# YuePanEdward/MULLS

Hardware: NVIDIA H100
Metric: scan-pair registrations/sec (120k-pt 64-beam) (higher is better)
Workload: dtype f32 geometry / f64 accumulation

## Files before the change

mulls_b200/csrc/kernels_ingest.cuh:

```cuda
#pragma once
#include "device_math.cuh"
#include "device_types.cuh"

namespace mulls {

template <bool kUndistort, bool kNormals>
__device__ __forceinline__ void load_input_point(const PairConst &pc, uint32_t seg, uint32_t local, float4 &pos, float4 &nrm) {
    const bool is_src = seg >= kNumClasses;
    const int cls = seg % kNumClasses;
    const bool undistort = kUndistort && is_src && pc.undistort && cls != MULLS_VERTEX;
    float x, y, z, intensity = 0.0f, curvature = 0.0f;
    float nx = 0.0f, ny = 0.0f, nz = 0.0f;
    const uint32_t fmt = pc.in_fmt[seg];
    if (fmt == 0u) {
        const float4 *in = pc.in_ptr[seg] + 3 * (size_t)local;
        const float4 a = in[0];
        x = a.x, y = a.y, z = a.z;
        if (kNormals) {
            const float4 b = in[1];
            const float4 c = in[2];
            nx = b.x, ny = b.y, nz = b.z;
            intensity = c.x, curvature = c.y;
        } else if (undistort) {
            curvature = reinterpret_cast<const float *>(in + 2)[1];
// ... 304 lines not shown
        uint32_t v = 0;
        if (i < total) v = A.ps[i / kNumSegs].seg_count[i % kNumSegs];
        uint32_t incl = v;
        for (int o = 1; o < 32; o <<= 1) {
            uint32_t t = __shfl_up_sync(0xffffffffu, incl, o);
            if ((threadIdx.x & 31) >= o) incl += t;
        }
        if ((threadIdx.x & 31) == 31) warp_sums[threadIdx.x >> 5] = incl;
        __syncthreads();
        if (threadIdx.x < 32) {
            uint32_t w = (threadIdx.x < (blockDim.x >> 5)) ? warp_sums[threadIdx.x] : 0;
            uint32_t wi = w;
            for (int o = 1; o < 32; o <<= 1) {
                uint32_t t = __shfl_up_sync(0xffffffffu, wi, o);
                if (threadIdx.x >= o) wi += t;
            }
            warp_sums[threadIdx.x] = wi - w;
        }
        __syncthreads();
        const uint32_t excl = carry + warp_sums[threadIdx.x >> 5] + incl - v;
        if (i < total) A.ps[i / kNumSegs].seg_start[i % kNumSegs] = excl;
        __syncthreads();
        if (threadIdx.x == blockDim.x - 1) carry = excl + v;
        __syncthreads();
    }
    for (int p = threadIdx.x; p < n_pairs; p += blockDim.x) {
        PairState &ps = A.ps[p];
        const PairConst &pc = A.pc[p];
        for (int c = 0; c < kNumClasses; ++c) {
            ps.n_tgt[c] = (int)ps.seg_count[c];
            ps.n_src[c] = (int)ps.seg_count[kNumClasses + c];
            ps.n_src_g[c] = ps.n_src[c];
            ps.n_corr[c] = 0;
            ps.n_corr_last[c] = 0;
        }
        int cnt = 0;
        if (pc.used[MULLS_PILLAR]) cnt += ps.n_src[MULLS_PILLAR];
        if (pc.used[MULLS_FACADE]) cnt += ps.n_src[MULLS_FACADE];
        if (pc.used[MULLS_BEAM]) cnt += ps.n_src[MULLS_BEAM];
        ps.source_feature_points_count = cnt;
    }
}

__device__ __forceinline__ int cell_top(const uint64_t *keys, uint32_t i, uint64_t kcur) {
    if (kcur == ~0ull || ((uint32_t)(kcur >> 36) % kNumSegs) >= kNumClasses) return -1;
    if (i == 0) return kMaxLevels - 1;
    const uint64_t kprev = keys[i - 1];
    if ((kprev >> 36) != (kcur >> 36)) return kMaxLevels - 1;
    const uint64_t diff = (kcur ^ kprev) & ((1ull << 36) - 1);
    if (diff == 0) return -1;
    return (63 - __clzll((long long)diff)) / 3;
}

template <bool kUndistort>
__global__ void __launch_bounds__(256) k_gather(DeviceArrays A, const uint64_t *keys, const uint32_t *vals, uint32_t n_total) {
    const uint32_t i = blockIdx.x * blockDim.x + threadIdx.x;
    const uint64_t key = i < n_total ? keys[i] : ~0ull;
    const uint32_t sg = (uint32_t)(key >> 36);
    const uint32_t pair = sg / kNumSegs, seg = sg % kNumSegs;
    const int top = cell_top(keys, i, key);
    const int cnt = top < 0 ? 0 : min(top, A.ps[pair].n_levels - 1) + 1;
    const bool is_tgt = key != ~0ull && seg < kNumClasses;
    const unsigned grp = __match_any_sync(0xffffffffu, is_tgt ? sg : 0xffffffffu);
    if (grp == 0xffffffffu) {
        const int tot = __reduce_add_sync(0xffffffffu, cnt);
        if ((threadIdx.x & 31) == 0 && tot > 0) atomicAdd(&A.ps[pair].hash_entries[seg], (unsigned)tot);
    } else if (cnt > 0) {
        atomicAdd(&A.ps[pair].hash_entries[seg], (unsigned)cnt);
    }
    if (key == ~0ull) return;
    const PairConst &pc = A.pc[pair];
    float4 pos, nrm;
    load_input_point<kUndistort, true>(pc, seg, vals[i] - pc.in_off[seg], pos, nrm);
    const uint32_t local = i - A.ps[pair].seg_start[seg];
    if (seg < kNumClasses) {
        const uint32_t d = pc.tgt_base[seg] + local;
        A.tgt_pos[d] = pos;
        A.tgt_nrm[d] = nrm;
    } else {
        const uint32_t d = pc.src_base[seg - kNumClasses] + local;
        if (pc.sharded) nrm.w = __int_as_float(__float_as_int(nrm.w) + (int)pc.src_index_base[seg - kNumClasses]);
        A.src_pos[0][d] = pos;
        A.src_nrm[0][d] = nrm;
        A.src_prevj[0][d] = -1;
        A.src_cert[0][d] = make_float4(0.f, 0.f, 0.f, 0.f);
    }
}

__device__ __forceinline__ void hash_insert(HashEntry *table, uint32_t hmask, uint32_t klo, uint32_t khi, uint32_t children,
                                            uint32_t start, uint32_t count) {
    uint32_t slot = cell_hash(klo, khi) & hmask;
    const unsigned long long packed = (unsigned long long)klo | ((unsigned long long)(khi | (children << 16)) << 32);
    while (true) {
        unsigned long long *kp = reinterpret_cast<unsigned long long *>(&table[slot]);
        if (atomicCAS(kp, 0ull, packed) == 0ull) {
            *reinterpret_cast<uint2 *>(&table[slot].start) = make_uint2(start, count);
            return;
        }
        slot = (slot + 1) & hmask;
    }
}

__device__ __forceinline__ uint32_t cell_end(const uint64_t *keys, uint32_t b, uint32_t hi, uint64_t p, int shift) {
    uint32_t in = b, out = hi, step = 1;
    while (in + step < hi) {
        if ((keys[in + step] >> shift) != p) {
            out = in + step;
            break;
        }
        in += step;
        step <<= 1;
    }
    while (out - in > 1) {
        const uint32_t mid = in + (out - in) / 2;
        if ((keys[mid] >> shift) == p) in = mid;
        else out = mid;
    }
    return out;
}

__global__ void __launch_bounds__(256) k_hash_build(DeviceArrays A, const uint64_t *keys, uint32_t n_total) {
    const uint32_t i = blockIdx.x * blockDim.x + threadIdx.x;
    if (i >= n_total || A.hash_used[1]) return;
    const uint64_t kcur = keys[i];
    const int top = cell_top(keys, i, kcur);
    if (top < 0) return;
    const uint32_t sg = (uint32_t)(kcur >> 36);
    const uint32_t pair = sg / kNumSegs, cls = sg % kNumSegs;
    const PairState &ps = A.ps[pair];
    const int L = ps.n_levels;
    const uint32_t seg_begin = ps.seg_start[cls], seg_end = seg_begin + ps.seg_count[cls];
    HashEntry *table = A.hash + ps.hash_base[cls];
    const uint32_t hmask = ps.hash_mask[cls];
    const uint64_t m = kcur & ((1ull << 36) - 1);
    const uint32_t x0 = compact12(m), y0 = compact12(m >> 1), z0 = compact12(m >> 2);
    uint32_t end = cell_end(keys, i, seg_end, kcur, 0);
    for (int l = 0; l <= top && l < L; ++l) {
        uint32_t children = 0;
        if (l > 0) {
            const int shift = 3 * l;
            const uint64_t p = kcur >> shift;
            children = 1u << ((kcur >> (shift - 3)) & 7u);
            while (end < seg_end) {
                const uint64_t k = keys[end];
                if ((k >> shift) != p) break;
                children |= 1u << ((k >> (shift - 3)) & 7u);
                end = cell_end(keys, end, seg_end, k >> (shift - 3), shift - 3);
            }
        }
        const uint32_t x = x0 >> l, y = y0 >> l, z = z0 >> l;
        hash_insert(table, hmask, cell_key_lo(x, y, z), cell_key_hi(z, l), children, i - seg_begin, end - i);
    }
}

constexpr uint64_t kHashSlack = 4;
__device__ __forceinline__ uint64_t hash_table_cap(int attempt, uint32_t cells) {
    const uint64_t want = (attempt == 0) ? kHashSlack * cells : (attempt == 1) ? 2ull * cells : (5ull * cells) / 4 + 1;
    uint64_t cap = 16;
    while (cap < want) cap <<= 1;
    return cap;
}
__global__ void k_hash_layout(DeviceArrays A, int n_pairs) {
    if (threadIdx.x != 0 || blockIdx.x != 0) return;
    for (int attempt = 0; attempt < 3; ++attempt) {
        uint64_t used = 0;
        bool overflow = false;
        for (int p = 0; p < n_pairs && !overflow; ++p) {
            PairState &ps = A.ps[p];
// ... 41 lines not shown
```

mulls_b200/csrc/kernels_iterate.cuh:

```cuda
#pragma once
#include <cooperative_groups.h>

#include "device_math.cuh"
#include "device_types.cuh"
#include "kernels_ingest.cuh"

namespace mulls {

__device__ __forceinline__ bool chunk_in_run(const DeviceArrays &A) { return blockIdx.x < (unsigned)A.ctl->n_it_chunks; }
__device__ __forceinline__ int loop_buf(const DeviceArrays &A, int buf) { return buf >= 0 ? buf : (A.ctl->it & 1); }
__device__ __forceinline__ mulls_icp_trace *trace_of(const DeviceArrays &A, uint32_t pair) {
    return (A.trace && A.ctl->trace_on) ? &A.trace[pair] : nullptr;
}

template <class Body>
__device__ __forceinline__ void for_each_live_chunk(const DeviceArrays &A, int parity, int which, Body body) {
    __shared__ uint32_t s_fetch;
    LoopCtl &ctl = *A.ctl;
    const uint32_t n = ctl.n_live[parity];
    const uint32_t *list = A.live_chunks + (size_t)parity * A.live_stride;
    for (;;) {
        __syncthreads();
        if (threadIdx.x == 0) s_fetch = atomicAdd(&ctl.work[which], 1u);
        __syncthreads();
        const uint32_t w = s_fetch;
        if (w >= n) break;
        body(list[w]);
    }
}

__device__ __forceinline__ void append_live_chunks(const DeviceArrays &A, int parity, uint32_t first, uint32_t count, uint32_t base) {
    uint32_t *list = A.live_chunks + (size_t)parity * A.live_stride;
    for (uint32_t k = threadIdx.x; k < count; k += blockDim.x) list[base + k] = first + k;
}

__global__ void __launch_bounds__(256) k_live_init(DeviceArrays A) {
    LoopCtl &ctl = *A.ctl;
    const uint32_t chunk = blockIdx.x * blockDim.x + threadIdx.x;
    bool live = false;
    if (chunk < (uint32_t)ctl.n_it_chunks) {
        const ChunkDesc cd = A.it_chunks[chunk];
        live = (int)cd.first < A.ps[cd.pair].n_src[cd.seg];
    }
    const unsigned m = __ballot_sync(0xffffffffu, live);
    if (!m) return;
    const int lane = threadIdx.x & 31;
    uint32_t base = 0;
    if (lane == 0) base = atomicAdd(&ctl.n_live[0], (unsigned)__popc(m));
    base = __shfl_sync(0xffffffffu, base, 0);
    if (live) A.live_chunks[base + __popc(m & ((1u << lane) - 1u))] = chunk;
}

constexpr int kStartLevel0 = 5;
constexpr int kLeafCount = 32;
constexpr int kDeferFromIter = 3;
constexpr float kReseedCells = 4.0f;

__device__ __forceinline__ GridView grid_of(const DeviceArrays &A, const PairConst &pc, const PairState &ps, int c) {
    GridView g;
    g.table = A.hash + ps.hash_base[c];
    g.mask = ps.hash_mask[c];
    g.pos = A.tgt_pos + pc.tgt_base[c];
    g.nrm = A.tgt_nrm + pc.tgt_base[c];
    g.ox = ps.origin[0], g.oy = ps.origin[1], g.oz = ps.origin[2];
    g.h0 = ps.h0, g.inv_h0 = ps.inv_h0;
    g.n_levels = ps.n_levels;
    g.leaf_count = kLeafCount;
    g.level_slack2 = 1.002001f;
    return g;
}

constexpr int kShootK = 10;

__device__ __forceinline__ void load_and_advance(DeviceArrays &A, const PairState &ps, int buf, uint32_t gi, bool valid,
                                                 float4 &p, float4 &n) {
    p = A.src_pos[buf][gi];
    n = A.src_nrm[buf][gi];
    if (valid && ps.iter > 0) {
        const double *t = ps.T_inc;
        const double px = p.x, py = p.y, pz = p.z, qx = n.x, qy = n.y, qz = n.z;
        p.x = (float)(t[0] * px + t[1] * py + t[2] * pz + t[3]);
        p.y = (float)(t[4] * px + t[5] * py + t[6] * pz + t[7]);
        p.z = (float)(t[8] * px + t[9] * py + t[10] * pz + t[11]);
        n.x = (float)(t[0] * qx + t[1] * qy + t[2] * qz);
        n.y = (float)(t[4] * qx + t[5] * qy + t[6] * qz);
        n.z = (float)(t[8] * qx + t[9] * qy + t[10] * qz);
        A.src_pos[buf][gi] = p;
        A.src_nrm[buf][gi] = n;
    }
}

__device__ __forceinline__ bool shoots(const PairConst &pc, int c) {
    return pc.normal_shooting && (c == MULLS_GROUND || c == MULLS_FACADE || c == MULLS_ROOF);
}

constexpr int kKeepFromIter = 3;

struct SearchFrame {
    GridView g;
    double max_dist_sqr;
    float r2_prune;
    bool defer;
};
__device__ __forceinline__ SearchFrame search_frame(const DeviceArrays &A, const PairConst &pc, const PairState &ps, int c) {
    SearchFrame f;
    f.g = grid_of(A, pc, ps, c);
    const float max_distance_f = 2.5f * ps.thre;
    f.max_dist_sqr = (double)max_distance_f * (double)max_distance_f;
    f.r2_prune = (float)f.max_dist_sqr * 1.0001f;
    f.defer = ps.iter >= kDeferFromIter;
    return f;
}

__device__ __forceinline__ void search_finish(DeviceArrays &A, const PairConst &pc, int c, uint32_t gi, int best_j, float best_d2,
                                              double max_dist_sqr, float orig_index_bits) {
    if (best_j >= 0 && !((double)best_d2 <= max_dist_sqr)) best_j = -1;
    if (best_j >= 0) {
        atomicMin(&A.claim[pc.tgt_base[c] + best_j], (unsigned)__float_as_int(orig_index_bits));
    }
    A.nn_idx[gi] = best_j;
    A.nn_d2[gi] = best_d2;
}

template <class Bounds>
__device__ __forceinline__ void search_one(DeviceArrays &A, const PairConst &pc, int c, int buf, uint32_t gi, const float4 p,
                                           float orig_bits, const SearchFrame &f, bool write_cert) {
    NoStats st;
    int best_j = -1;
    float best_d2 = INFINITY;
    const int pj = A.src_prevj[buf][gi];
    if (pj >= 0) {
        const float4 q = __ldg(&f.g.pos[pj]);
        best_d2 = flann_l2(p.x, p.y, p.z, q.x, q.y, q.z);
        best_j = pj;
    }
    {
        const float rs = kReseedCells * f.g.h0;
        if (best_j < 0 || best_d2 > rs * rs) {
            float d2 = INFINITY;
            int j = -1;
            walk_greedy_seed(f.g, p.x, p.y, p.z, kStartLevel0, d2, j, st);
            if (j >= 0 && d2 < best_d2) best_d2 = d2, best_j = j;
        }
    }
    const float cert2 = nn_search_walk_b<Bounds>(f.g, p.x, p.y, p.z, f.r2_prune, kStartLevel0, f.defer, best_d2, best_j, st);
    if (write_cert) A.src_cert[buf][gi] = make_float4(p.x, p.y, p.z, sqrtf(cert2));
    search_finish(A, pc, c, gi, best_j, best_d2, f.max_dist_sqr, orig_bits);
}

template <class Bounds>
__device__ __forceinline__ void search_quarter(DeviceArrays &A, int buf, uint32_t chunk, uint32_t sub, bool write_cert) {
    const ChunkDesc cd = A.it_chunks[chunk];
    const PairConst &pc = A.pc[cd.pair];
    const PairState &ps = A.ps[cd.pair];
    if (ps.status != kRunning || A.hash_used[1]) return;
    const int c = (int)cd.seg;
    const int ns = ps.n_src[c], nt = ps.n_tgt[c], nsg = ps.n_src_g[c];
    if ((int)cd.first >= ns) return;
    if (shoots(pc, c)) return;
    const uint32_t local = cd.first + 32u * sub + (threadIdx.x & 31u);
    const bool valid = (int)local < ns;
    const uint32_t gi = pc.src_base[c] + (valid ? local : 0);
    float4 p, n;
    load_and_advance(A, ps, buf, gi, valid, p, n);
    if (!valid) return;
    if (!(pc.used[c] && nsg >= 3 && nt >= 3)) {
        A.nn_idx[gi] = -1;
        A.nn_d2[gi] = INFINITY;
        return;
    }
    const SearchFrame f = search_frame(A, pc, ps, c);
    search_one<Bounds>(A, pc, c, buf, gi, p, n.w, f, write_cert);
}

__device__ __forceinline__ void search_keep_chunk(DeviceArrays &A, int buf, uint32_t chunk, uint8_t *need_list, uint32_t *n_need) {
    const ChunkDesc cd = A.it_chunks[chunk];
    const PairConst &pc = A.pc[cd.pair];
    const PairState &ps = A.ps[cd.pair];
    if (ps.status != kRunning || A.hash_used[1]) return;
    const int c = (int)cd.seg;
    const int ns = ps.n_src[c], nt = ps.n_tgt[c], nsg = ps.n_src_g[c];
    if ((int)cd.first >= ns) return;
    if (shoots(pc, c)) return;
    const int lane = threadIdx.x & 31;
    const bool active = pc.used[c] && nsg >= 3 && nt >= 3;
    const SearchFrame f = search_frame(A, pc, ps, c);
    if (threadIdx.x == 0) *n_need = 0u;
    __syncthreads();
    {
        const uint32_t local = cd.first + threadIdx.x;
        const bool valid = (int)local < ns;
        const uint32_t gi = pc.src_base[c] + (valid ? local : 0);
        float4 p, n;
        load_and_advance(A, ps, buf, gi, valid, p, n);
        bool need = false;
        if (valid) {
            if (!active) {
                A.nn_idx[gi] = -1;
                A.nn_d2[gi] = INFINITY;
            } else {
                need = true;
                const int pj = A.src_prevj[buf][gi];
                const float4 ce = A.src_cert[buf][gi];
                if (pj >= 0 && ce.w > 0.0f) {
                    const float4 q = __ldg(&f.g.pos[pj]);
                    const float d1 = flann_l2(p.x, p.y, p.z, q.x, q.y, q.z);
                    const float mv = flann_l2(p.x, p.y, p.z, ce.x, ce.y, ce.z);
                    if ((sqrtf(d1) + sqrtf(mv)) * 1.0001f + 3e-5f < ce.w * 0.9999f) {
                        search_finish(A, pc, c, gi, pj, d1, f.max_dist_sqr, n.w);
                        need = false;
                    }
                }
            }
        }
        const unsigned m = __ballot_sync(0xffffffffu, need);
        uint32_t base = 0;
        if (lane == 0 && m) base = atomicAdd(n_need, (uint32_t)__popc(m));
        base = __shfl_sync(0xffffffffu, base, 0);
        if (need) need_list[base + __popc(m & ((1u << lane) - 1u))] = (uint8_t)threadIdx.x;
    }
    __syncthreads();
    if (threadIdx.x < *n_need) {
        const uint32_t gi = pc.src_base[c] + cd.first + need_list[threadIdx.x];
        const float4 p = A.src_pos[buf][gi];
        search_one<WalkBounds>(A, pc, c, buf, gi, p, A.src_nrm[buf][gi].w, f, true);
    }
}

constexpr int kSearchBlocksPerSm = 10;
__device__ __forceinline__ int search_mode_of(int it) { return it >= kKeepFromIter ? 2 : (it == kKeepFromIter - 1 ? 1 : 0); }

template <int kMode>
__global__ void __launch_bounds__(kIterBlock, kSearchBlocksPerSm) k_search(DeviceArrays A, int buf, int it) {
    buf = loop_buf(A, buf);
    if (it < 0) it = A.ctl->it;
    if (blockIdx.x == 0 && threadIdx.x == 0) {
        LoopCtl &ctl = *A.ctl;
        ctl.work[1] = ctl.work[2] = ctl.work[3] = 0u;
        ctl.n_live[buf ^ 1] = 0u;
    }
    if (search_mode_of(it) != kMode) return;
    if (kMode == 2) {
        __shared__ uint8_t s_need[kIterBlock];
        __shared__ uint32_t s_n_need;
        for_each_live_chunk(A, buf, 0, [&](uint32_t chunk) { search_keep_chunk(A, buf, chunk, s_need, &s_n_need); });
    } else {
        const uint32_t n_units = (kIterBlock / 32) * A.ctl->n_live[buf];
        const uint32_t *list = A.live_chunks + (size_t)buf * A.live_stride;
        for (;;) {
            uint32_t u = 0;
            if ((threadIdx.x & 31) == 0) u = atomicAdd(&A.ctl->work[0], 1u);
            u = __shfl_sync(0xffffffffu, u, 0);
            if (u >= n_units) break;
            if (kMode == 1) search_quarter<WalkBounds>(A, buf, list[u / (kIterBlock / 32)], u % (kIterBlock / 32), true);
            else search_quarter<NoBounds>(A, buf, list[u / (kIterBlock / 32)], u % (kIterBlock / 32), false);
            __syncwarp();
        }
    }
}

__device__ __forceinline__ void search_shoot_chunk(DeviceArrays &A, int buf, uint32_t chunk) {
    const ChunkDesc cd = A.it_chunks[chunk];
    const PairConst &pc = A.pc[cd.pair];
    const PairState &ps = A.ps[cd.pair];
    if (ps.status != kRunning || A.hash_used[1]) return;
    const int c = (int)cd.seg;
    const int ns = ps.n_src[c], nt = ps.n_tgt[c], nsg = ps.n_src_g[c];
    if ((int)cd.first >= ns || !shoots(pc, c)) return;
    const uint32_t local = cd.first + threadIdx.x;
    const bool valid = (int)local < ns;
    const uint32_t gi = pc.src_base[c] + (valid ? local : 0);
    float4 p, n;
    load_and_advance(A, ps, buf, gi, valid, p, n);
    if (!valid) return;
    if (!(pc.used[c] && nsg >= 3 && nt >= 3)) {
        A.nn_idx[gi] = -1;
        A.nn_d2[gi] = INFINITY;
        return;
    }
    const GridView g = grid_of(A, pc, ps, c);
    const float max_distance_f = 2.5f * ps.thre;
    int sj = -1;
    float sd2 = INFINITY;
    KnnList<kShootK> kl;
    knn_search(g, p.x, p.y, p.z, kStartLevel0, kShootK, kl);
    double min_dist = 1.7976931348623157e308;
    for (int t = 0; t < kl.n; ++t) {
        const float4 q = __ldg(&g.pos[kl.j[t]]);
        const float ptx = q.x - p.x, pty = q.y - p.y, ptz = q.z - p.z;
        const double Nx = n.x, Ny = n.y, Nz = n.z, Vx = ptx, Vy = pty, Vz = ptz;
        const double Cx = Ny * Vz - Nz * Vy, Cy = Nz * Vx - Nx * Vz, Cz = Nx * Vy - Ny * Vx;
        const double dist = Cx * Cx + (Cy * Cy + Cz * Cz);
        if (dist < min_dist) {
            min_dist = dist;
            sj = kl.j[t];
            sd2 = kl.d2[t];
        }
    }
    if (sj >= 0 && min_dist > (double)max_distance_f) sj = -1;
    if (sj >= 0) atomicMin(&A.claim[pc.tgt_base[c] + sj], (unsigned)__float_as_int(n.w));
    A.nn_idx[gi] = sj;
    A.nn_d2[gi] = sd2;
}
__global__ void __launch_bounds__(kIterBlock) k_search_shoot(DeviceArrays A, int buf) {
    buf = loop_buf(A, buf);
    for_each_live_chunk(A, buf, 3, [&](uint32_t chunk) { search_shoot_chunk(A, buf, chunk); });
}

__device__ __forceinline__ void resolve_body(DeviceArrays &A, int buf, uint32_t chunk) {
    const ChunkDesc cd = A.it_chunks[chunk];
    const PairConst &pc = A.pc[cd.pair];
    PairState &ps = A.ps[cd.pair];
    if (ps.status != kRunning) return;
    const int c = (int)cd.seg;
    const int ns = ps.n_src[c], nt = ps.n_tgt[c], nsg = ps.n_src_g[c];
    const uint32_t local = cd.first + threadIdx.x;
    const bool valid = (int)local < ns;
    const bool active = pc.used[c] && nsg >= 3 && nt >= 3;
    const bool dedup = active && nsg >= kDedupMinSrc;
    bool kept = false, pass = false;
    if (valid) {
        const uint32_t gi = pc.src_base[c] + local;
        const int j = A.nn_idx[gi];
        const bool matched = active && j >= 0;
        bool corr = matched;
        kept = true;
        if (dedup) {
            const float4 n = A.src_nrm[buf][gi];
            const bool winner = matched && A.claim[pc.tgt_base[c] + j] == (unsigned)__float_as_int(n.w);
            kept = winner;
            corr = winner;
        }
        if (corr) {
            const float d2 = A.nn_d2[gi];
            pass = d2 < ps.thre * ps.thre;
            if (pass && c != MULLS_VERTEX) {
                const float4 n = A.src_nrm[buf][gi];
                const float4 m = A.tgt_nrm[pc.tgt_base[c] + j];
                const double dot = (double)n.x * (double)m.x + (double)n.y * (double)m.y + (double)n.z * (double)m.z;
                const float cos_angle = (float)fabs(dot);
                if ((double)cos_angle < pc.cos_thre) pass = false;
            }
        }
        A.flags[gi] = (uint8_t)((kept ? 1 : 0) | (pass ? 2 : 0));
    }
    const unsigned kb = __ballot_sync(0xffffffffu, kept);
    const unsigned pb = __ballot_sync(0xffffffffu, pass);
    __shared__ unsigned s_kept[kIterBlock / 32], s_pass[kIterBlock / 32];
    if ((threadIdx.x & 31) == 0) {
        s_kept[threadIdx.x >> 5] = __popc(kb);
        s_pass[threadIdx.x >> 5] = __popc(pb);
    }
    __syncthreads();
    if (threadIdx.x == 0) {
        unsigned k = 0, p = 0;
        for (int w = 0; w < kIterBlock / 32; ++w) {
            k += s_kept[w];
            p += s_pass[w];
        }
        A.blk_kept[chunk] = k;
        if (p) atomicAdd(&ps.n_corr[c], p);
    }
}
__global__ void __launch_bounds__(kIterBlock) k_resolve(DeviceArrays A, int buf) {
    buf = loop_buf(A, buf);
    for_each_live_chunk(A, buf, 1, [&](uint32_t chunk) { resolve_body(A, buf, chunk); });
}

template <class Sink>
__device__ __forceinline__ void terms_pt2pl(const float4 p, const float pi, const float4 q, const float4 qn,
                                            float weight, int iter_num, bool dist_w, bool resid_w, bool inten_w,
                                            float window, Sink t, float &w_out) {
    const float px = p.x, py = p.y, pz = p.z, qx = q.x, qy = q.y, qz = q.z;
    const float ntx = qn.x, nty = qn.y, ntz = qn.z;
    float w = weight;
    const float a = ntz * py - nty * pz;
    const float b = ntx * pz - ntz * px;
    const float c = nty * px - ntx * py;
    const float d = ntx * qx + nty * qy + ntz * qz - ntx * px - nty * py - ntz * pz;
    const float dist = sqrtf(qx * qx + qy * qy + qz * qz);
    if (dist_w) w = w * weight_by_dist_adaptive(dist, iter_num);
    if (resid_w) w = w * weight_by_residual(fabsf(d), window);
    if (inten_w) w = w * weight_by_intensity((float)((double)pi + 0.0001), (float)((double)q.w + 0.0001));
    w_out = w;
    t[0] = w * ntx * ntx;
    t[1] = w * ntx * nty;
    t[2] = w * ntx * ntz;
    t[3] = w * a * ntx;
    t[4] = w * b * ntx;
    t[5] = w * c * ntx;
    t[6] = w * nty * nty;
    t[7] = w * nty * ntz;
    t[8] = w * a * nty;
    t[9] = w * b * nty;
    t[10] = w * c * nty;
    t[11] = w * ntz * ntz;
    t[12] = w * a * ntz;
    t[13] = w * b * ntz;
    t[14] = w * c * ntz;
    t[15] = w * a * a;
    t[16] = w * a * b;
    t[17] = w * a * c;
    t[18] = w * b * b;
    t[19] = w * b * c;
    t[20] = w * c * c;
    t[21] = w * d * ntx;
    t[22] = w * d * nty;
    t[23] = w * d * ntz;
    t[24] = w * d * a;
    t[25] = w * d * b;
    t[26] = w * d * c;
}

__device__ __forceinline__ int diag_index(int j) {
    const int d[6] = {0, 6, 11, 15, 18, 20};
    return d[j];
}

template <class Sink>
__device__ __forceinline__ void terms_pt2li(const float4 p, const float pi, const float4 q, const float4 qv,
                                            float weight, int iter_num, bool dist_w, bool resid_w, bool inten_w,
                                            float window, Sink t, float &w_out) {
    const float px = p.x, py = p.y, pz = p.z, qx = q.x, qy = q.y, qz = q.z;
    const float vx = qv.x, vy = qv.y, vz = qv.z;
    const float dx = px - qx, dy = py - qy, dz = pz - qz;
    double Am[3][6], bv[3];
    Am[0][0] = 0;
    Am[0][1] = (double)(-vz);
    Am[0][2] = (double)vy;
    Am[0][3] = (double)(vy * py + vz * pz);
    Am[0][4] = (double)(-vy * px);
    Am[0][5] = (double)(-vz * px);
    Am[1][0] = (double)vz;
    Am[1][1] = 0;
    Am[1][2] = (double)(-vx);
    Am[1][3] = (double)(-vx * py);
    Am[1][4] = (double)(vz * pz + vx * px);
    Am[1][5] = (double)(-vz * py);
    Am[2][0] = (double)(-vy);
    Am[2][1] = (double)vx;
    Am[2][2] = 0;
    Am[2][3] = (double)(-vx * pz);
    Am[2][4] = (double)(-vy * pz);
    Am[2][5] = (double)(vx * px + vy * py);
    bv[0] = (double)(-vy * dz + vz * dy);
    bv[1] = (double)(-vz * dx + vx * dz);
    bv[2] = (double)(-vx * dy + vy * dx);
// ... 180 lines not shown
        for (int r = 0; r < 3; ++r)
            for (int cc = 0; cc < 3; ++cc)
                cof[6 * (3 + r) + cc] = J[r][0] * inv[6 * 3 + cc] + J[r][1] * inv[6 * 4 + cc] + J[r][2] * inv[6 * 5 + cc];
    }
    double *Tt = ps.T_inc;
    construct_trans_a(x, Tt);
    const double ts_norm = sqrt(Tt[3] * Tt[3] + Tt[7] * Tt[7] + Tt[11] * Tt[11]);
    const double rs_angle = fabs(rotation_angle(Tt));
    if (ts_norm > (double)pc.max_t || rs_angle > (double)pc.max_r) {
        ps.code = -1;
        ps.status = kDone;
        pair_left_running(A);
        return;
    }
    mat4_mul(Tt, ps.T_total, Tmp);
    for (int k = 0; k < 16; ++k) ps.T_total[k] = Tmp[k];
    if (i == pc.max_iter - 1 || (i > 2 && ts_norm < (double)pc.conv_t && rs_angle < (double)pc.conv_r)) {
        ps.status = kNeedPosterior;
        ps.final_buf = buf_written;
        pair_left_running(A);
        return;
    }
    ps.iter = i + 1;
}

__device__ __forceinline__ void accumulate_body(DeviceArrays &A, int buf, uint32_t chunk) {
    const ChunkDesc cd = A.it_chunks[chunk];
    const PairConst &pc = A.pc[cd.pair];
    PairState &ps = A.ps[cd.pair];
    if (ps.status != kRunning) return;
    const int c = (int)cd.seg;
    const int ns = ps.n_src[c];
    const uint32_t local = cd.first + threadIdx.x;
    const bool valid = (int)local < ns;
    const int lane = threadIdx.x & 31, warp = threadIdx.x >> 5;
    constexpr int kWarps = kIterBlock / 32;
    __shared__ double s_terms[27 * kIterBlock];
    __shared__ uint32_t s_off[kWarps + 1];
    __shared__ uint32_t s_base;

    if ((int)cd.first >= ns) return;
    uint32_t dst_local = 0;
    uint8_t fl = 0;
    uint32_t gi = 0;
    bool kept = false, pass = false;
    struct Column {
        double *base;
        __device__ __forceinline__ double &operator[](int k) const { return base[k * kIterBlock]; }
    } t = {s_terms + threadIdx.x};
    {
        uint32_t acc = 0;
        const uint32_t first_chunk = pc.class_chunk_begin[c];
        for (uint32_t b = first_chunk + threadIdx.x; b < chunk; b += kIterBlock) acc += A.blk_kept[b];
        for (int o = 16; o > 0; o >>= 1) acc += __shfl_xor_sync(0xffffffffu, acc, o);
        if (lane == 0) s_off[warp] = acc;
        __syncthreads();
        if (threadIdx.x == 0) {
            uint32_t tt = 0;
            for (int w = 0; w < kWarps; ++w) tt += s_off[w];
            s_base = tt;
        }
        __syncthreads();
    }
    if (valid) {
        gi = pc.src_base[c] + local;
        fl = A.flags[gi];
    }
    kept = (fl & 1) != 0, pass = (fl & 2) != 0;
    const unsigned kb = __ballot_sync(0xffffffffu, kept);
    if (lane == 0) s_off[warp] = __popc(kb);
    __syncthreads();
    if (threadIdx.x == 0) {
        uint32_t run = 0;
        for (int w = 0; w < kWarps; ++w) {
            const uint32_t tt = s_off[w];
            s_off[w] = run;
            run += tt;
        }
        s_off[kWarps] = run;
    }
    __syncthreads();
    dst_local = s_base + s_off[warp] + __popc(kb & ((1u << lane) - 1u));

    float w_store = 0.0f;
    int j = -1;
    float4 p = make_float4(0, 0, 0, 0), n = make_float4(0, 0, 0, 0);
    float d2 = 0.0f;
    if (valid) {
        p = A.src_pos[buf][gi];
        n = A.src_nrm[buf][gi];
        j = A.nn_idx[gi];
        d2 = A.nn_d2[gi];
        if (j >= 0) A.claim[pc.tgt_base[c] + j] = kClaimFree;
    }
    uint32_t n_corr[kNumClasses];
#pragma unroll
    for (int k = 0; k < kNumClasses; ++k) n_corr[k] = ps.n_corr[k];
    float ratio_unused;
    const bool few = too_few(pc, ps, n_corr, ratio_unused);
    if (pass && !few) {
        const float4 q = A.tgt_pos[pc.tgt_base[c] + j];
        const float4 qn = A.tgt_nrm[pc.tgt_base[c] + j];
        const int it = ps.iter;
        const bool resid_w = pc.w_residual && it > 2;
        const bool dist_w = pc.w_dist != 0, inten_w = pc.w_intensity != 0;
        if (c == MULLS_GROUND || c == MULLS_FACADE || c == MULLS_ROOF) {
            const float wc = (c == MULLS_FACADE) ? 1.0f : balanced_ground_weight(pc, n_corr);
            terms_pt2pl(p, p.w, q, qn, wc, it, dist_w, resid_w, inten_w, pc.win_pt2pl, t, w_store);
        } else if (c == MULLS_PILLAR || c == MULLS_BEAM) {
            terms_pt2li(p, p.w, q, qn, 1.0f, it, dist_w, resid_w, inten_w, pc.win_pt2li, t, w_store);
        } else {
            terms_pt2pt(p, p.w, q, 1.0f, it, dist_w, resid_w, inten_w, pc.win_pt2pt, t);
            w_store = d2;
        }
    } else {
#pragma unroll
        for (int k = 0; k < 27; ++k) t[k] = 0.0;
    }
    if (kept) {
        const uint32_t gd = pc.src_base[c] + dst_local;
        A.src_pos[buf ^ 1][gd] = p;
        A.src_nrm[buf ^ 1][gd] = n;
        A.src_prevj[buf ^ 1][gd] = j;
        A.src_cert[buf ^ 1][gd] = A.src_cert[buf][gi];
        A.corr_j[gd] = pass ? j : -1;
        A.corr_w[gd] = w_store;
    }
    __syncthreads();
#pragma unroll 1
    for (int k = warp; k < 27; k += kWarps) {
        const double *row = s_terms + k * kIterBlock;
        double v = ((row[lane] + row[lane + 32]) + row[lane + 64]) + row[lane + 96];
#pragma unroll
        for (int o = 16; o > 0; o >>= 1) v += __shfl_xor_sync(0xffffffffu, v, o);
        if (lane == 0) A.partials[(size_t)chunk * kTerms + k] = v;
    }
}
__global__ void __launch_bounds__(kIterBlock, 8) k_accumulate(DeviceArrays A, int buf) {
    buf = loop_buf(A, buf);
    if (blockIdx.x == 0 && threadIdx.x == 0) A.ctl->work[0] = 0u;
    for_each_live_chunk(A, buf, 2, [&](uint32_t chunk) { accumulate_body(A, buf, chunk); });
}

__device__ __forceinline__ void publish_live_chunks(const DeviceArrays &A, uint32_t pair, int next_parity) {
    __shared__ uint32_t s_base;
    __syncthreads();
    const PairConst &pc = A.pc[pair];
    const PairState &ps = A.ps[pair];
    if (ps.status != kRunning) return;
    uint32_t count[kNumClasses], total = 0;
#pragma unroll
    for (int c = 0; c < kNumClasses; ++c) {
        count[c] = (uint32_t)((ps.n_src[c] + kIterBlock - 1) / kIterBlock);
        total += count[c];
    }
    if (threadIdx.x == 0) s_base = atomicAdd(&A.ctl->n_live[next_parity], total);
    __syncthreads();
    uint32_t base = s_base;
#pragma unroll
    for (int c = 0; c < kNumClasses; ++c) {
        append_live_chunks(A, next_parity, pc.class_chunk_begin[c], count[c], base);
        base += count[c];
    }
}

__device__ __forceinline__ void solve_body(DeviceArrays &A, int buf, uint32_t pair) {
    const PairConst &pc = A.pc[pair];
    PairState &ps = A.ps[pair];
    if (ps.status != kRunning) return;
    const int lane = threadIdx.x & 31, warp = threadIdx.x >> 5, n_warps = blockDim.x >> 5;
    __shared__ double s_S[kNumClasses][kTerms];
    __shared__ double s_scratch[160];
    __shared__ int s_newn[kNumClasses];
    __shared__ uint32_t s_ncorr[kNumClasses];
    for (int cc = warp; cc < kNumClasses; cc += n_warps) {
        const uint32_t b0 = pc.class_chunk_begin[cc];
        const uint32_t live = (uint32_t)((ps.n_src[cc] + kIterBlock - 1) / kIterBlock);
        const uint32_t b1 = min(pc.class_chunk_begin[cc + 1], b0 + live);
        double a0 = 0.0, a1 = 0.0, a2 = 0.0, a3 = 0.0;
        if (lane < 27) {
            uint32_t b = b0;
            for (; b + 4 <= b1; b += 4) {
                a0 += A.partials[(size_t)(b + 0) * kTerms + lane];
                a1 += A.partials[(size_t)(b + 1) * kTerms + lane];
                a2 += A.partials[(size_t)(b + 2) * kTerms + lane];
                a3 += A.partials[(size_t)(b + 3) * kTerms + lane];
            }
            for (; b < b1; ++b) a0 += A.partials[(size_t)b * kTerms + lane];
        }
        if (lane < kTerms) s_S[cc][lane] = (lane < 27) ? ((a0 + a1) + (a2 + a3)) : 0.0;
        uint32_t acc = 0;
        for (uint32_t b = b0 + lane; b < b1; b += 32) acc += A.blk_kept[b];
        for (int o = 16; o > 0; o >>= 1) acc += __shfl_xor_sync(0xffffffffu, acc, o);
        if (lane == 0) {
            s_newn[cc] = (int)acc;
            s_ncorr[cc] = ps.n_corr[cc];
        }
    }
    __syncthreads();
    if (threadIdx.x == 0) {
        uint64_t srcpts = 0;
        for (int cc = 0; cc < kNumClasses; ++cc)
            if (pc.used[cc]) srcpts += (uint64_t)ps.n_src_g[cc];
        ps.alg_bytes += 28ull * srcpts;
        if (pc.sharded) {
            for (int cc = 0; cc < kNumClasses; ++cc) {
                ps.n_src[cc] = s_newn[cc];
                for (int k = 0; k < kTerms; ++k) A.xch_f64[cc * kTerms + k] = (k < 27) ? s_S[cc][k] : 0.0;
            }
        } else {
        mulls_icp_trace *tr = trace_of(A, pair);
        for (int cc = 0; cc < kNumClasses; ++cc) {
            ps.n_src[cc] = s_newn[cc];
            ps.n_src_g[cc] = s_newn[cc];
            ps.n_corr[cc] = s_ncorr[cc];
            if (tr && ps.iter < MULLS_MAX_TRACE_ITERS) tr->n_src[ps.iter][cc] = (uint32_t)ps.n_src[cc];
        }
        solve_and_advance(A, pair, &s_S[0][0], s_scratch, buf ^ 1);
        for (int cc = 0; cc < kNumClasses; ++cc) ps.n_corr[cc] = 0;
        }
    }
    if (!pc.sharded) publish_live_chunks(A, pair, buf ^ 1);
}
constexpr int kSolveThreads = kNumClasses * 32;
__global__ void __launch_bounds__(kSolveThreads) k_solve(DeviceArrays A, int buf, unsigned long long loop_handle) {
    LoopCtl &ctl = *A.ctl;
    if (blockIdx.x >= (unsigned)ctl.n_pairs) return;
    solve_body(A, loop_buf(A, buf), blockIdx.x);
    if (loop_handle == 0ull) return;
    __syncthreads();
    if (threadIdx.x == 0) {
        __threadfence();
        if (atomicAdd(&ctl.solved, 1u) == (unsigned)ctl.n_pairs - 1u) {
            ctl.solved = 0;
            const int it = ctl.it + 1;
            ctl.it = it;
            __threadfence();
            const bool again = *(volatile int *)A.running > 0 && it < ctl.max_iter;
            cudaGraphSetConditional((cudaGraphConditionalHandle)loop_handle, again ? 1u : 0u);
        }
    }
}

__global__ void __launch_bounds__(kIterBlock, 4) k_icp_loop(DeviceArrays A) {
    namespace cg = cooperative_groups;
    cg::grid_group grid = cg::this_grid();
    LoopCtl &ctl = *A.ctl;
    __shared__ uint8_t s_need[kIterBlock];
    __shared__ uint32_t s_n_need;
    const int n_pairs = ctl.n_pairs, max_iter = ctl.max_iter;
    for (int it = 0; it < max_iter; ++it) {
        const int buf = it & 1;
        const uint32_t *list = A.live_chunks + (size_t)buf * A.live_stride;
        const uint32_t n_live = ctl.n_live[buf];
        if (blockIdx.x == 0 && threadIdx.x == 0) ctl.n_live[buf ^ 1] = 0u;
        for (uint32_t w = blockIdx.x; w < n_live; w += gridDim.x) {
            const uint32_t chunk = list[w];
            if (it >= kKeepFromIter) search_keep_chunk(A, buf, chunk, s_need, &s_n_need);
            else if (it == kKeepFromIter - 1) search_quarter<WalkBounds>(A, buf, chunk, threadIdx.x >> 5, true);
            else search_quarter<NoBounds>(A, buf, chunk, threadIdx.x >> 5, false);
            __syncthreads();
        }
        grid.sync();
        for (uint32_t w = blockIdx.x; w < n_live; w += gridDim.x) {
            resolve_body(A, buf, list[w]);
            __syncthreads();
        }
        grid.sync();
        for (uint32_t w = blockIdx.x; w < n_live; w += gridDim.x) {
            accumulate_body(A, buf, list[w]);
            __syncthreads();
        }
        grid.sync();
        for (int pair = blockIdx.x; pair < n_pairs; pair += gridDim.x) {
            solve_body(A, buf, (uint32_t)pair);
            __syncthreads();
        }
        grid.sync();
        if (*(volatile int *)A.running <= 0) break;
    }
}

__global__ void k_shard_pack_setup(DeviceArrays A, int phase) {
    PairState &ps = A.ps[0];
    if (phase == 0) {
        for (int d = 0; d < 3; ++d) {
            A.xch_i32[d] = ps.bb_src[d];
            A.xch_i32[3 + d] = ~ps.bb_src[3 + d];
        }
    } else if (phase == 1) {
        for (int d = 0; d < 3; ++d) {
            ps.bb_src[d] = A.xch_i32[d];
            ps.bb_src[3 + d] = ~A.xch_i32[3 + d];
        }
    } else if (phase == 2) {
        for (int c = 0; c < kNumClasses; ++c) A.xch_i32[c] = ps.n_src[c];
    } else {
        const PairConst &pc = A.pc[0];
        int cnt = 0;
        for (int c = 0; c < kNumClasses; ++c) ps.n_src_g[c] = A.xch_i32[c];
        if (pc.used[MULLS_PILLAR]) cnt += ps.n_src_g[MULLS_PILLAR];
        if (pc.used[MULLS_FACADE]) cnt += ps.n_src_g[MULLS_FACADE];
        if (pc.used[MULLS_BEAM]) cnt += ps.n_src_g[MULLS_BEAM];
        ps.source_feature_points_count = cnt;
    }
}
__global__ void __launch_bounds__(kIterBlock) k_shard_counts(DeviceArrays A, int phase) {
    const PairConst &pc = A.pc[0];
    PairState &ps = A.ps[0];
    if (ps.status != kRunning) {
        if (phase == 0 && threadIdx.x < 2 * kNumClasses) A.xch_i32[threadIdx.x] = 0;
        return;
    }
    if (phase == 0) {
        __shared__ uint32_t s_w[kIterBlock / 32];
        for (int cc = 0; cc < kNumClasses; ++cc) {
            const uint32_t b0 = pc.class_chunk_begin[cc];
            const uint32_t live = (uint32_t)((ps.n_src[cc] + kIterBlock - 1) / kIterBlock);
            const uint32_t b1 = min(pc.class_chunk_begin[cc + 1], b0 + live);
            uint32_t acc = 0;
            for (uint32_t b = b0 + threadIdx.x; b < b1; b += kIterBlock) acc += A.blk_kept[b];
            for (int o = 16; o > 0; o >>= 1) acc += __shfl_xor_sync(0xffffffffu, acc, o);
            __syncthreads();
            if ((threadIdx.x & 31) == 0) s_w[threadIdx.x >> 5] = acc;
            __syncthreads();
            if (threadIdx.x == 0) {
                uint32_t tot = 0;
                for (int w = 0; w < kIterBlock / 32; ++w) tot += s_w[w];
                A.xch_i32[kNumClasses + cc] = (int)tot;
                A.xch_i32[cc] = (int)ps.n_corr[cc];
            }
        }
    } else if (threadIdx.x == 0) {
        for (int cc = 0; cc < kNumClasses; ++cc) {
            ps.n_corr[cc] = (uint32_t)A.xch_i32[cc];
            ps.n_src_g_next[cc] = A.xch_i32[kNumClasses + cc];
        }
    }
}
__global__ void k_shard_solve(DeviceArrays A, int buf, int it_flag) {
    PairState &ps = A.ps[0];
// ... 230 lines not shown
```

mulls_b200/csrc/mulls_b200.cu:

```cuda
#include <algorithm>
#include <atomic>
#include <memory>
#include <cmath>
#include <cstdio>
#include <chrono>
#include <cstring>
#include <string>
#include <vector>

#include <cub/device/device_radix_sort.cuh>
#include <cub/device/device_scan.cuh>
#include <cub/device/device_select.cuh>

#include <dlfcn.h>
#include <mutex>

#include "device_types.cuh"
#include "host_pack.h"
#include "scan_io.h"
#include "kernels_ingest.cuh"
#include "kernels_iterate.cuh"
#include "kernels_pca.cuh"
#include "kernels_map.cuh"
#include "kernels_classify.cuh"
// ... 695 lines not shown
    CK(cudaMemsetAsync(A.claim, 0x7f, std::max<size_t>(ctx->n_tgt_total, 1) * sizeof(unsigned), st));
    k_state_init<<<(unsigned)ceil_div(np, 128), 128, 0, st>>>(A, np);
    ++launches;
    const unsigned n_inc = (unsigned)ctx->h_in_chunks.size();
    if (n_inc) {
        if (ctx->any_undistort) k_ingest_bbox<true><<<n_inc, kIngestBlock, 0, st>>>(A);
        else if (finite_only) k_ingest_bbox<false, true><<<n_inc, kIngestBlock, 0, st>>>(A);
        else k_ingest_bbox<false><<<n_inc, kIngestBlock, 0, st>>>(A);
        ++launches;
    }
    if (hook) {
        k_shard_pack_setup<<<1, 1, 0, st>>>(A, 0);
        if (hook(user, A.xch_i32, 6, 1, 1, (void *)st) != 0) {
            ctx->err = "all-reduce callback failed";
            return MULLS_E_COMM;
        }
        k_shard_pack_setup<<<1, 1, 0, st>>>(A, 1);
        launches += 2;
    }
    k_pair_setup<<<(unsigned)ceil_div(np, 128), 128, 0, st>>>(A, np);
    ++launches;
    if (n_inc) {
        if (ctx->any_undistort) k_make_keys<true><<<n_inc, kIngestBlock, 0, st>>>(A);
        else if (finite_only) k_make_keys<false, true><<<n_inc, kIngestBlock, 0, st>>>(A);
        else k_make_keys<false><<<n_inc, kIngestBlock, 0, st>>>(A);
        ++launches;
        if (ctx->any_keep_less) {
            const unsigned pb = (unsigned)ceil_div(np, 64);
            k_keepless_plan<<<pb, 64, 0, st>>>(A, np);
            for (int pass = 0; pass < 8; ++pass) {
                k_keepless_hist<<<n_inc, kIngestBlock, 0, st>>>(A, pass);
                k_keepless_step<<<pb, 64, 0, st>>>(A, np, pass);
            }
            k_keepless_mark<<<n_inc, kIngestBlock, 0, st>>>(A);
            launches += 18;
        }
        int seg_bits = 1;
        while ((1ull << seg_bits) <= (uint64_t)np * kNumSegs) ++seg_bits;
        size_t bytes = ctx->cub_temp_bytes;
        CK(cub::DeviceRadixSort::SortPairs(ctx->cub_temp, bytes, A.keys_a, A.keys_b, A.vals_a, A.vals_b, (int)n_in, 0,
                                           36 + seg_bits, st));
    }
    k_seg_offsets<<<1, 256, 0, st>>>(A, np);
    ++launches;
    if (hook) {
        k_shard_pack_setup<<<1, 1, 0, st>>>(A, 2);
        if (hook(user, A.xch_i32, kNumClasses, 1, 0, (void *)st) != 0) {
            ctx->err = "all-reduce callback failed";
            return MULLS_E_COMM;
        }
        k_shard_pack_setup<<<1, 1, 0, st>>>(A, 3);
        launches += 2;
    }
    if (n_in) {
        const unsigned nb = (unsigned)ceil_div(n_in, 256);
        if (ctx->any_undistort) k_gather<true><<<nb, 256, 0, st>>>(A, A.keys_b, A.vals_b, n_in);
        else k_gather<false><<<nb, 256, 0, st>>>(A, A.keys_b, A.vals_b, n_in);
        k_hash_layout<<<1, 32, 0, st>>>(A, np);
        k_hash_clear<<<1184, 256, 0, st>>>(A);
        k_hash_build<<<nb, 256, 0, st>>>(A, A.keys_b, n_in);
        launches += 4;
    } else {
        k_hash_layout<<<1, 32, 0, st>>>(A, np);
        ++launches;
    }
    return MULLS_OK;
}

static unsigned chunk_bucket(const mulls_ctx *ctx) {
    unsigned b = 1;
    while (b < (unsigned)ctx->h_it_chunks.size()) b <<= 1;
    return b;
}
static unsigned resident_grid(const mulls_ctx *ctx, int blocks_per_sm) {
    return std::min((unsigned)(ctx->num_sms * blocks_per_sm), chunk_bucket(ctx));
}
static void launch_search(mulls_ctx *ctx, cudaStream_t st, const DeviceArrays &A, int buf, int it) {
    const unsigned grid = resident_grid(ctx, kSearchBlocksPerSm);
    const int mode = it < 0 ? -1 : (it >= kKeepFromIter ? 2 : (it == kKeepFromIter - 1 ? 1 : 0));
    if (mode < 0 || mode == 0) k_search<0><<<grid, kIterBlock, 0, st>>>(A, buf, it);
    if (mode < 0 || mode == 1) k_search<1><<<grid, kIterBlock, 0, st>>>(A, buf, it);
    if (mode < 0 || mode == 2) k_search<2><<<grid, kIterBlock, 0, st>>>(A, buf, it);
}
constexpr int kShootBlocksPerSm = 8, kResolveBlocksPerSm = 16, kAccumulateBlocksPerSm = 8;
constexpr int kPollPause = 64;

static int build_iteration_graph(mulls_ctx *ctx) {
    const int key[2] = {(int)chunk_bucket(ctx), ctx->any_normal_shooting ? 1 : 0};
    if (ctx->graph_exec && std::memcmp(key, ctx->graph_key, sizeof(key)) == 0) return MULLS_OK;
    if (ctx->graph_exec) cudaGraphExecDestroy(ctx->graph_exec), ctx->graph_exec = nullptr;
    if (ctx->graph) cudaGraphDestroy(ctx->graph), ctx->graph = nullptr;
    cudaStream_t st = ctx->stream;
    DeviceArrays A = ctx->A;
    const unsigned cap_chunks = (unsigned)std::max<size_t>(ctx->cap_it_chunks, 1), cap_pairs = (unsigned)std::max<size_t>(ctx->max_pairs, 1);
    CK(cudaGraphCreate(&ctx->graph, 0));
    cudaGraphConditionalHandle handle;
    CK(cudaGraphConditionalHandleCreate(&handle, ctx->graph, 1, cudaGraphCondAssignDefault));
    cudaGraphNodeParams wp = {cudaGraphNodeTypeConditional};
    wp.conditional.handle = handle;
    wp.conditional.type = cudaGraphCondTypeWhile;
    wp.conditional.size = 1;
    cudaGraphNode_t while_node;
    CK(cudaGraphAddNode(&while_node, ctx->graph, nullptr, 0, &wp));
    cudaGraph_t body = wp.conditional.phGraph_out[0];
    CK(cudaStreamBeginCaptureToGraph(st, body, nullptr, nullptr, 0, cudaStreamCaptureModeThreadLocal));
    launch_search(ctx, st, A, -1, -1);
    if (ctx->any_normal_shooting)
        k_search_shoot<<<resident_grid(ctx, kShootBlocksPerSm), kIterBlock, 0, st>>>(A, -1);
    k_resolve<<<resident_grid(ctx, kResolveBlocksPerSm), kIterBlock, 0, st>>>(A, -1);
    k_accumulate<<<resident_grid(ctx, kAccumulateBlocksPerSm), kIterBlock, 0, st>>>(A, -1);
    k_solve<<<cap_pairs, kSolveThreads, 0, st>>>(A, -1, (unsigned long long)handle);
    CK(cudaStreamEndCapture(st, nullptr));
    CK(cudaStreamBeginCaptureToGraph(st, ctx->graph, &while_node, nullptr, 1, cudaStreamCaptureModeThreadLocal));
    k_posterior<<<std::min(cap_chunks, chunk_bucket(ctx)), kIterBlock, 0, st>>>(A);
    k_finalize<<<(unsigned)ceil_div(cap_pairs, 64), 64, 0, st>>>(A, -1);
    k_collect<<<(unsigned)ceil_div(cap_pairs, 128), 128, 0, st>>>(A, -1, ctx->d_results);
    CK(cudaStreamEndCapture(st, nullptr));
    CK(cudaGraphInstantiate(&ctx->graph_exec, ctx->graph, 0));
    std::memcpy(ctx->graph_key, key, sizeof(key));
    return MULLS_OK;
}

static int grow_hash_pool(mulls_ctx *ctx) {
    const uint32_t need = ctx->h_flags[2];
    DeviceArrays &A = ctx->A;
    if (need <= A.hash_pool_entries || need == 0xffffffffu) {
        ctx->err = "hash pool exhausted (the target clouds need " + std::to_string(need) + " grid entries)";
        return MULLS_E_CAPACITY;
    }
    HashEntry *fresh = nullptr;
    if (cudaMalloc(&fresh, (size_t)need * sizeof(HashEntry)) != cudaSuccess) {
        cudaGetLastError();
        ctx->err = "hash pool exhausted, and no device memory to grow it to " + std::to_string(need) + " entries";
        return MULLS_E_CAPACITY;
    }
    std::replace(ctx->allocs.begin(), ctx->allocs.end(), (void *)A.hash, (void *)fresh);
    CK(cudaFree(A.hash));
    A.hash = fresh;
    A.hash_pool_entries = need;
    if (ctx->graph_exec) cudaGraphExecDestroy(ctx->graph_exec), ctx->graph_exec = nullptr;
    if (ctx->graph) cudaGraphDestroy(ctx->graph), ctx->graph = nullptr;
    return MULLS_OK;
}

static int run_impl_inner(mulls_ctx *ctx, mulls_icp_result *out, mulls_icp_trace *trace, mulls_allreduce_fn hook, void *user,
                          bool finish_now);
static int run_finish_inner(mulls_ctx *ctx, mulls_icp_result *out);
static int run_impl(mulls_ctx *ctx, mulls_icp_result *out, mulls_icp_trace *trace, mulls_allreduce_fn hook, void *user,
                    bool finish_now = true) {
    const int rc = run_impl_inner(ctx, out, trace, hook, user, finish_now);
    if (rc != MULLS_OK && ctx && ctx->stream) cudaStreamSynchronize(ctx->stream);
    return rc;
}
static int run_finish(mulls_ctx *ctx, mulls_icp_result *out) {
    const int rc = run_finish_inner(ctx, out);
    if (rc != MULLS_OK && ctx && ctx->stream) cudaStreamSynchronize(ctx->stream);
    return rc;
}
static int run_impl_inner(mulls_ctx *ctx, mulls_icp_result *out, mulls_icp_trace *trace, mulls_allreduce_fn hook, void *user,
                          bool finish_now) {
    if (!ctx || !ctx->uploaded) return MULLS_E_ARG;
    ctx->pend.active = false;
    CK(cudaSetDevice(ctx->device));
    cudaStream_t st = ctx->stream;
    DeviceArrays A = ctx->A;
    const int np = (int)ctx->n_pairs;
    uint64_t launches = 0;
// ... 1832 lines not shown
```

Measured before the change: 6144.

## Defer incremental transform to compaction pass instead of writing back in search

Search and shoot kernels no longer write transformed source points and normals back to global memory. They apply the incremental transform on the fly in registers, and the accumulate/compaction step writes the advanced pos/nrm into the next buffer. The keep-chunk search carries the transformed point through shared memory to avoid reloading it. Ingest no longer initialises prevj/cert, and the iteration index now gates their use. Cert is copied only from the keep iteration onward, and resolve gets explicit launch bounds. This cuts global read-modify-write traffic per iteration, at the cost of recomputing the transform in several kernels and a subtle dependency on iteration gating for correctness.

```diff
diff --git a/mulls_b200/csrc/kernels_ingest.cuh b/mulls_b200/csrc/kernels_ingest.cuh
--- a/mulls_b200/csrc/kernels_ingest.cuh
+++ b/mulls_b200/csrc/kernels_ingest.cuh
@@ -410,8 +410,6 @@
         if (pc.sharded) nrm.w = __int_as_float(__float_as_int(nrm.w) + (int)pc.src_index_base[seg - kNumClasses]);
         A.src_pos[0][d] = pos;
         A.src_nrm[0][d] = nrm;
-        A.src_prevj[0][d] = -1;
-        A.src_cert[0][d] = make_float4(0.f, 0.f, 0.f, 0.f);
     }
 }
 
diff --git a/mulls_b200/csrc/kernels_iterate.cuh b/mulls_b200/csrc/kernels_iterate.cuh
--- a/mulls_b200/csrc/kernels_iterate.cuh
+++ b/mulls_b200/csrc/kernels_iterate.cuh
@@ -72,22 +72,25 @@
 
 constexpr int kShootK = 10;
 
-__device__ __forceinline__ void load_and_advance(DeviceArrays &A, const PairState &ps, int buf, uint32_t gi, bool valid,
-                                                 float4 &p, float4 &n) {
-    p = A.src_pos[buf][gi];
-    n = A.src_nrm[buf][gi];
-    if (valid && ps.iter > 0) {
+__device__ __forceinline__ float4 advanced_pos(const PairState &ps, float4 p) {
+    if (ps.iter > 0) {
         const double *t = ps.T_inc;
-        const double px = p.x, py = p.y, pz = p.z, qx = n.x, qy = n.y, qz = n.z;
+        const double px = p.x, py = p.y, pz = p.z;
         p.x = (float)(t[0] * px + t[1] * py + t[2] * pz + t[3]);
         p.y = (float)(t[4] * px + t[5] * py + t[6] * pz + t[7]);
         p.z = (float)(t[8] * px + t[9] * py + t[10] * pz + t[11]);
+    }
+    return p;
+}
+__device__ __forceinline__ float4 advanced_nrm(const PairState &ps, float4 n) {
+    if (ps.iter > 0) {
+        const double *t = ps.T_inc;
+        const double qx = n.x, qy = n.y, qz = n.z;
         n.x = (float)(t[0] * qx + t[1] * qy + t[2] * qz);
         n.y = (float)(t[4] * qx + t[5] * qy + t[6] * qz);
         n.z = (float)(t[8] * qx + t[9] * qy + t[10] * qz);
-        A.src_pos[buf][gi] = p;
-        A.src_nrm[buf][gi] = n;
-    }
+    }
+    return n;
 }
 
 __device__ __forceinline__ bool shoots(const PairConst &pc, int c) {
@@ -124,11 +127,11 @@
 
 template <class Bounds>
 __device__ __forceinline__ void search_one(DeviceArrays &A, const PairConst &pc, int c, int buf, uint32_t gi, const float4 p,
-                                           float orig_bits, const SearchFrame &f, bool write_cert) {
+                                           float orig_bits, const SearchFrame &f, bool write_cert, bool seeded) {
     NoStats st;
     int best_j = -1;
     float best_d2 = INFINITY;
-    const int pj = A.src_prevj[buf][gi];
+    const int pj = seeded ? A.src_prevj[buf][gi] : -1;
     if (pj >= 0) {
         const float4 q = __ldg(&f.g.pos[pj]);
         best_d2 = flann_l2(p.x, p.y, p.z, q.x, q.y, q.z);
@@ -159,21 +162,20 @@
     if ((int)cd.first >= ns) return;
     if (shoots(pc, c)) return;
     const uint32_t local = cd.first + 32u * sub + (threadIdx.x & 31u);
-    const bool valid = (int)local < ns;
-    const uint32_t gi = pc.src_base[c] + (valid ? local : 0);
-    float4 p, n;
-    load_and_advance(A, ps, buf, gi, valid, p, n);
-    if (!valid) return;
+    if ((int)local >= ns) return;
+    const uint32_t gi = pc.src_base[c] + local;
     if (!(pc.used[c] && nsg >= 3 && nt >= 3)) {
         A.nn_idx[gi] = -1;
         A.nn_d2[gi] = INFINITY;
         return;
     }
+    const float4 p = advanced_pos(ps, A.src_pos[buf][gi]);
     const SearchFrame f = search_frame(A, pc, ps, c);
-    search_one<Bounds>(A, pc, c, buf, gi, p, n.w, f, write_cert);
-}
-
-__device__ __forceinline__ void search_keep_chunk(DeviceArrays &A, int buf, uint32_t chunk, uint8_t *need_list, uint32_t *n_need) {
+    search_one<Bounds>(A, pc, c, buf, gi, p, A.src_nrm[buf][gi].w, f, write_cert, ps.iter > 0);
+}
+
+__device__ __forceinline__ void search_keep_chunk(DeviceArrays &A, int buf, uint32_t chunk, uint8_t *need_list, float4 *carry,
+                                                  uint32_t *n_need) {
     const ChunkDesc cd = A.it_chunks[chunk];
     const PairConst &pc = A.pc[cd.pair];
     const PairState &ps = A.ps[cd.pair];
@@ -191,8 +193,7 @@
         const uint32_t local = cd.first + threadIdx.x;
         const bool valid = (int)local < ns;
         const uint32_t gi = pc.src_base[c] + (valid ? local : 0);
-        float4 p, n;
-        load_and_advance(A, ps, buf, gi, valid, p, n);
+        float4 p = make_float4(0.f, 0.f, 0.f, 0.f);
         bool need = false;
         if (valid) {
             if (!active) {
@@ -200,6 +201,8 @@
                 A.nn_d2[gi] = INFINITY;
             } else {
                 need = true;
+                p = advanced_pos(ps, A.src_pos[buf][gi]);
+                p.w = A.src_nrm[buf][gi].w;
                 const int pj = A.src_prevj[buf][gi];
                 const float4 ce = A.src_cert[buf][gi];
                 if (pj >= 0 && ce.w > 0.0f) {
@@ -207,7 +210,7 @@
                     const float d1 = flann_l2(p.x, p.y, p.z, q.x, q.y, q.z);
                     const float mv = flann_l2(p.x, p.y, p.z, ce.x, ce.y, ce.z);
                     if ((sqrtf(d1) + sqrtf(mv)) * 1.0001f + 3e-5f < ce.w * 0.9999f) {
-                        search_finish(A, pc, c, gi, pj, d1, f.max_dist_sqr, n.w);
+                        search_finish(A, pc, c, gi, pj, d1, f.max_dist_sqr, p.w);
                         need = false;
                     }
                 }
@@ -217,13 +220,17 @@
         uint32_t base = 0;
         if (lane == 0 && m) base = atomicAdd(n_need, (uint32_t)__popc(m));
         base = __shfl_sync(0xffffffffu, base, 0);
-        if (need) need_list[base + __popc(m & ((1u << lane) - 1u))] = (uint8_t)threadIdx.x;
+        if (need) {
+            const uint32_t k = base + __popc(m & ((1u << lane) - 1u));
+            need_list[k] = (uint8_t)threadIdx.x;
+            carry[k] = p;
+        }
     }
     __syncthreads();
     if (threadIdx.x < *n_need) {
         const uint32_t gi = pc.src_base[c] + cd.first + need_list[threadIdx.x];
-        const float4 p = A.src_pos[buf][gi];
-        search_one<WalkBounds>(A, pc, c, buf, gi, p, A.src_nrm[buf][gi].w, f, true);
+        const float4 p = carry[threadIdx.x];
+        search_one<WalkBounds>(A, pc, c, buf, gi, p, p.w, f, true, true);
     }
 }
 
@@ -242,8 +249,9 @@
     if (search_mode_of(it) != kMode) return;
     if (kMode == 2) {
         __shared__ uint8_t s_need[kIterBlock];
+        __shared__ float4 s_carry[kIterBlock];
         __shared__ uint32_t s_n_need;
-        for_each_live_chunk(A, buf, 0, [&](uint32_t chunk) { search_keep_chunk(A, buf, chunk, s_need, &s_n_need); });
+        for_each_live_chunk(A, buf, 0, [&](uint32_t chunk) { search_keep_chunk(A, buf, chunk, s_need, s_carry, &s_n_need); });
     } else {
         const uint32_t n_units = (kIterBlock / 32) * A.ctl->n_live[buf];
         const uint32_t *list = A.live_chunks + (size_t)buf * A.live_stride;
@@ -268,16 +276,14 @@
     const int ns = ps.n_src[c], nt = ps.n_tgt[c], nsg = ps.n_src_g[c];
     if ((int)cd.first >= ns || !shoots(pc, c)) return;
     const uint32_t local = cd.first + threadIdx.x;
-    const bool valid = (int)local < ns;
-    const uint32_t gi = pc.src_base[c] + (valid ? local : 0);
-    float4 p, n;
-    load_and_advance(A, ps, buf, gi, valid, p, n);
-    if (!valid) return;
+    if ((int)local >= ns) return;
+    const uint32_t gi = pc.src_base[c] + local;
     if (!(pc.used[c] && nsg >= 3 && nt >= 3)) {
         A.nn_idx[gi] = -1;
         A.nn_d2[gi] = INFINITY;
         return;
     }
+    const float4 p = advanced_pos(ps, A.src_pos[buf][gi]), n = advanced_nrm(ps, A.src_nrm[buf][gi]);
     const GridView g = grid_of(A, pc, ps, c);
     const float max_distance_f = 2.5f * ps.thre;
     int sj = -1;
@@ -326,8 +332,8 @@
         bool corr = matched;
         kept = true;
         if (dedup) {
-            const float4 n = A.src_nrm[buf][gi];
-            const bool winner = matched && A.claim[pc.tgt_base[c] + j] == (unsigned)__float_as_int(n.w);
+            const float orig = A.src_nrm[buf][gi].w;
+            const bool winner = matched && A.claim[pc.tgt_base[c] + j] == (unsigned)__float_as_int(orig);
             kept = winner;
             corr = winner;
         }
@@ -335,7 +341,7 @@
             const float d2 = A.nn_d2[gi];
             pass = d2 < ps.thre * ps.thre;
             if (pass && c != MULLS_VERTEX) {
-                const float4 n = A.src_nrm[buf][gi];
+                const float4 n = advanced_nrm(ps, A.src_nrm[buf][gi]);
                 const float4 m = A.tgt_nrm[pc.tgt_base[c] + j];
                 const double dot = (double)n.x * (double)m.x + (double)n.y * (double)m.y + (double)n.z * (double)m.z;
                 const float cos_angle = (float)fabs(dot);
@@ -362,7 +368,8 @@
         if (p) atomicAdd(&ps.n_corr[c], p);
     }
 }
-__global__ void __launch_bounds__(kIterBlock) k_resolve(DeviceArrays A, int buf) {
+constexpr int kResolveBlocksPerSm = 16;
+__global__ void __launch_bounds__(kIterBlock, kResolveBlocksPerSm) k_resolve(DeviceArrays A, int buf) {
     buf = loop_buf(A, buf);
     for_each_live_chunk(A, buf, 1, [&](uint32_t chunk) { resolve_body(A, buf, chunk); });
 }
@@ -709,17 +716,21 @@
     __syncthreads();
     dst_local = s_base + s_off[warp] + __popc(kb & ((1u << lane) - 1u));
 
-    float w_store = 0.0f;
+    float4 p = make_float4(0, 0, 0, 0);
     int j = -1;
-    float4 p = make_float4(0, 0, 0, 0), n = make_float4(0, 0, 0, 0);
     float d2 = 0.0f;
-    if (valid) {
-        p = A.src_pos[buf][gi];
-        n = A.src_nrm[buf][gi];
+    const uint32_t gd = pc.src_base[c] + dst_local;
+    if (kept) {
+        p = advanced_pos(ps, A.src_pos[buf][gi]);
         j = A.nn_idx[gi];
         d2 = A.nn_d2[gi];
         if (j >= 0) A.claim[pc.tgt_base[c] + j] = kClaimFree;
-    }
+        A.src_pos[buf ^ 1][gd] = p;
+        A.src_nrm[buf ^ 1][gd] = advanced_nrm(ps, A.src_nrm[buf][gi]);
+        A.src_prevj[buf ^ 1][gd] = j;
+        if (ps.iter >= kKeepFromIter - 1) A.src_cert[buf ^ 1][gd] = A.src_cert[buf][gi];
+    }
+    float w_store = 0.0f;
     uint32_t n_corr[kNumClasses];
 #pragma unroll
     for (int k = 0; k < kNumClasses; ++k) n_corr[k] = ps.n_corr[k];
@@ -745,11 +756,6 @@
         for (int k = 0; k < 27; ++k) t[k] = 0.0;
     }
     if (kept) {
-        const uint32_t gd = pc.src_base[c] + dst_local;
-        A.src_pos[buf ^ 1][gd] = p;
-        A.src_nrm[buf ^ 1][gd] = n;
-        A.src_prevj[buf ^ 1][gd] = j;
-        A.src_cert[buf ^ 1][gd] = A.src_cert[buf][gi];
         A.corr_j[gd] = pass ? j : -1;
         A.corr_w[gd] = w_store;
     }
@@ -874,6 +880,7 @@
     cg::grid_group grid = cg::this_grid();
     LoopCtl &ctl = *A.ctl;
     __shared__ uint8_t s_need[kIterBlock];
+    __shared__ float4 s_carry[kIterBlock];
     __shared__ uint32_t s_n_need;
     const int n_pairs = ctl.n_pairs, max_iter = ctl.max_iter;
     for (int it = 0; it < max_iter; ++it) {
@@ -883,7 +890,7 @@
         if (blockIdx.x == 0 && threadIdx.x == 0) ctl.n_live[buf ^ 1] = 0u;
         for (uint32_t w = blockIdx.x; w < n_live; w += gridDim.x) {
             const uint32_t chunk = list[w];
-            if (it >= kKeepFromIter) search_keep_chunk(A, buf, chunk, s_need, &s_n_need);
+            if (it >= kKeepFromIter) search_keep_chunk(A, buf, chunk, s_need, s_carry, &s_n_need);
             else if (it == kKeepFromIter - 1) search_quarter<WalkBounds>(A, buf, chunk, threadIdx.x >> 5, true);
             else search_quarter<NoBounds>(A, buf, chunk, threadIdx.x >> 5, false);
             __syncthreads();
diff --git a/mulls_b200/csrc/mulls_b200.cu b/mulls_b200/csrc/mulls_b200.cu
--- a/mulls_b200/csrc/mulls_b200.cu
+++ b/mulls_b200/csrc/mulls_b200.cu
@@ -801,7 +801,7 @@
     if (mode < 0 || mode == 1) k_search<1><<<grid, kIterBlock, 0, st>>>(A, buf, it);
     if (mode < 0 || mode == 2) k_search<2><<<grid, kIterBlock, 0, st>>>(A, buf, it);
 }
-constexpr int kShootBlocksPerSm = 8, kResolveBlocksPerSm = 16, kAccumulateBlocksPerSm = 8;
+constexpr int kShootBlocksPerSm = 8, kAccumulateBlocksPerSm = 8;
 constexpr int kPollPause = 64;
 
 static int build_iteration_graph(mulls_ctx *ctx) {
```

Result: faster. 6337, median of 6 (+3.2%).
